# cambyse/po-rrt

Measured on NVIDIA B200. Metric: edge_world_validity_checks_per_s, higher is better.
Workload: dtype u8

## Files before the change

### po_rrt_b200/csrc/common.cuh

```cuda
#pragma once
#include <cuda_runtime.h>
#include <stdint.h>

#include <cstdio>
#include <cstring>
#include <string>
#include <vector>

#include "../../include/porrt_b200.h"

#define PORRT_API extern "C" __attribute__((visibility("default")))

struct DevBuf {
  void* p = nullptr;
  size_t cap = 0;
  cudaError_t ensure(size_t bytes) {
    if (bytes <= cap) return cudaSuccess;
    if (p) cudaFree(p);
    p = nullptr; cap = 0;
    size_t want = bytes + bytes / 4 + 256;
    cudaError_t e = cudaMalloc(&p, want);
    if (e == cudaSuccess) cap = want;
    return e;
  }
  cudaError_t grow_keep(size_t bytes, size_t keep_bytes, cudaStream_t st) {
    if (bytes <= cap) return cudaSuccess;
    void* q = nullptr;
    const size_t want = bytes + bytes / 2 + 256;
    cudaError_t e = cudaMalloc(&q, want);
    if (e != cudaSuccess) return e;
    if (p && keep_bytes) {
      e = cudaMemcpyAsync(q, p, keep_bytes, cudaMemcpyDeviceToDevice, st);
      if (e == cudaSuccess) e = cudaStreamSynchronize(st);
      if (e != cudaSuccess) { cudaFree(q); return e; }
    }
    if (p) cudaFree(p);
    p = q; cap = want;
    return cudaSuccess;
  }
  void release() { if (p) cudaFree(p); p = nullptr; cap = 0; }
  template <class T> T* as() const { return (T*)p; }
};

struct PinBuf {
  void* p = nullptr;
  size_t cap = 0;
  cudaError_t ensure(size_t bytes) {
    if (bytes <= cap) return cudaSuccess;
    if (p) cudaFreeHost(p);
    p = nullptr; cap = 0;
    size_t want = bytes + bytes / 4 + 256;
    cudaError_t e = cudaHostAlloc(&p, want, cudaHostAllocDefault);
    if (e == cudaSuccess) cap = want;
    return e;
  }
  void release() { if (p) cudaFreeHost(p); p = nullptr; cap = 0; }
  template <class T> T* as() const { return (T*)p; }
};

struct MapDev {
  const uint8_t* grid;
  const uint8_t* coarse;
  int32_t coarse_cw;
  const uint32_t* plane;
  const uint32_t* bits;
  int32_t plane_cw, plane_ch;
  int32_t plane_bytes;
  int32_t plane_guard;
  int32_t bits_var_words;
  int32_t H, W;
  int32_t tiles_x;
  int32_t kind;
  int32_t free_vid;
  int32_t mask_words;
  double low0, low1, ppm, hm1;
};

static const int MAX_SLOTS = 3;

struct porrt_ctx {
  int device = 0;
  int sm_count = 148;
  cudaStream_t stream = nullptr;
  cudaStream_t own_stream = nullptr;
  cudaStream_t copy_in = nullptr, copy_out = nullptr;
  cudaEvent_t ev_in[MAX_SLOTS] = {}, ev_k[MAX_SLOTS] = {}, ev_out[MAX_SLOTS] = {};
  std::string err;
  int64_t launches = 0;
  cudaEvent_t ev_t[16] = {};
  int n_marks = 0, n_last = 0;
  double last_ms[16] = {};

  bool has_map = false;
  MapDev map = {};
  int n_zones = 0, n_worlds = 0, n_validities = 0, mask_words = 1;
  double visibility = 0.0;
  std::vector<uint64_t> validities;
  std::vector<double> zone_pos;
  std::vector<uint64_t> zone_world_masks;
  DevBuf d_grid, d_coarse, d_validities, d_zone_pos, d_plane, d_bits;
  bool force_large_map_path = false;
  bool force_global_sweeps = false;

  int64_t n_vertices = 0;
  bool grid_stale = false;
  double cell_request = 0.0;
  double cell = 0, inv_cell = 0, org_x = 0, org_y = 0;
  int32_t cells_x = 0, cells_y = 0;
  DevBuf d_vxy_sorted, d_vid_sorted, d_cell_start, d_vxy, d_vcell;
  DevBuf nn_tmp[3];
  DevBuf d_nbr_start, d_nbr_script;
  bool nbr_ready = false;
  DevBuf nn_stage;
  DevBuf comm_tmp;
  DevBuf nn_stage2;
  int32_t nn_fb_n = 0;
  int32_t reach_words = 1;

  struct BeliefState_ {
    int64_t V = 0; int32_t B = 0, n_worlds = 0;
    std::vector<int64_t> row_ptr; std::vector<int32_t> col, edge_vid; std::vector<double> xy;
    std::vector<double> beliefs;
    const double* dist = nullptr; const uint8_t* type = nullptr;
    std::vector<uint8_t> exists;
    std::vector<int32_t> node_obs_set;
    std::vector<int64_t> succ_ptr;
    std::vector<int32_t> succ_belief;
    std::vector<uint8_t> compat;
    int32_t n_validities = 0;
    bool on_host = false;
    DevBuf dev;
    const double* d_dist_cm = nullptr; const uint8_t* d_type_cm = nullptr; const uint8_t* d_type = nullptr; const int32_t* d_colpos = nullptr;
    std::vector<int32_t> colpos;
    std::vector<std::vector<double>> col_dist;
    std::vector<std::vector<uint8_t>> col_type;
  } bel;
  std::vector<int32_t> bel_node_vid;
  DevBuf d_bel_succ;
  int64_t prm_n = 0, prm_edges = 0;
  const int64_t* prm_row_ptr = nullptr;
  const int32_t* prm_col = nullptr;
  const void* radii_ptr = nullptr; int64_t radii_lo = 0, radii_n = 0; double radii_ms = 0, radii_sr = 0;
  DevBuf d_prm_row, d_prm_col;

  struct MmPrm_ {
    std::vector<int64_t> row_ptr; std::vector<int32_t> col, belief_id; std::vector<uint8_t> type;
  } mm;

  void* comm = nullptr;
  int comm_rank = 0, comm_world = 1;

  DevBuf kd_buf;
  cudaStream_t aux_stream = nullptr;
  DevBuf scratch[12];
  PinBuf pin[6];
  PinBuf pin_flags;
};

#define CTX_CHECK(ctx) do { if (!(ctx)) return PORRT_ERR_INVALID_ARG; } while (0)

static inline int32_t porrt_fail(porrt_ctx* ctx, int32_t code, const std::string& msg) {
  if (ctx) ctx->err = msg;
  return code;
}

#define CUDA_TRY(ctx, expr)                                                                        \
  do {                                                                                             \
    cudaError_t _e = (expr);                                                                       \
    if (_e != cudaSuccess) {                                                                       \
      char _b[512];                                                                                \
      snprintf(_b, sizeof(_b), "%s:%d %s -> %s", __FILE__, __LINE__, #expr, cudaGetErrorString(_e)); \
      return porrt_fail(ctx, PORRT_ERR_CUDA, _b);                                                  \
    }                                                                                              \
  } while (0)

#define LAUNCH_CHECK(ctx)                                                                          \
  do {                                                                                             \
    (ctx)->launches += 1;                                                                          \
    CUDA_TRY(ctx, cudaGetLastError());                                                             \
  } while (0)

static inline bool is_pinned_host(const void* p) {
  cudaPointerAttributes a;
  if (cudaPointerGetAttributes(&a, p) != cudaSuccess) { cudaGetLastError(); return false; }
  return a.type == cudaMemoryTypeHost;
}

static inline void tstart(porrt_ctx* ctx) { ctx->n_marks = 0; if (ctx->ev_t[0]) cudaEventRecord(ctx->ev_t[ctx->n_marks++], ctx->stream); }
static inline void tmark(porrt_ctx* ctx) { if (ctx->ev_t[0] && ctx->n_marks < 16) cudaEventRecord(ctx->ev_t[ctx->n_marks++], ctx->stream); }
static inline void tfinish(porrt_ctx* ctx) {
  ctx->n_last = 0;
  for (int k = 0; k + 1 < ctx->n_marks; ++k) {
    float ms = 0.f;
    if (cudaEventElapsedTime(&ms, ctx->ev_t[k], ctx->ev_t[k + 1]) != cudaSuccess) { cudaGetLastError(); ms = -1.f; }
    ctx->last_ms[ctx->n_last++] = ms;
  }
}

static inline int div_up(int64_t a, int64_t b) { return (int)((a + b - 1) / b); }

void comm_shard_range(int64_t n, int rank, int world, int64_t* lo, int64_t* hi);
int32_t comm_all_gatherv_dev(porrt_ctx* ctx, const void* send_dev, void* recv_dev, const int64_t* offsets , cudaStream_t st);
struct EdgeOut {
  int32_t* vid = nullptr;
  int8_t* vid8 = nullptr;
  uint64_t* mask = nullptr;
};
int32_t map_edge_validity_dev(porrt_ctx* ctx, const double* from_dev, const double* to_dev, int64_t n,
                              int32_t* out_vid_dev, uint64_t* out_mask_dev, cudaStream_t st);
int32_t map_edge_launch(porrt_ctx* ctx, const double* from_dev, const double* to_dev, const int32_t* from_idx_dev,
                        const int32_t* to_idx_dev, int64_t n, const EdgeOut& out, cudaStream_t st);
int32_t map_edge_validity_indexed_dev(porrt_ctx* ctx, const double* xy_dev, const int32_t* from_idx_dev, const int32_t* to_idx_dev,
                                      int64_t n, int32_t* out_vid_dev, cudaStream_t st);
int32_t edge3_build(porrt_ctx* ctx, cudaStream_t st);
bool edge3_usable(const porrt_ctx* ctx);
int32_t edge3_launch(porrt_ctx* ctx, const double* from_dev, const double* to_dev, int64_t n, const EdgeOut& out,
                     const int32_t* from_idx_dev, const int32_t* to_idx_dev, cudaStream_t st);
struct GridDev;
bool nn_tile_usable(const porrt_ctx* ctx, int64_t m);
int32_t nn_tile_radius_collect(porrt_ctx* ctx, const GridDev& g, const double* q_dev, const double* radius_dev, int64_t m,
                               const uint32_t* prefix_dev, const uint64_t* reach_dev, const uint32_t* world_dev, int32_t* counts_dev,
                               int64_t* stg_off_dev, const int32_t** staging_out, const int32_t** fb_list_out, int32_t* fb_n_out,
                               int64_t* staged_total_out = nullptr);
int32_t nn_tile_radius_place(porrt_ctx* ctx, const int32_t* staging, const int64_t* stg_off_dev, const int64_t* offsets_dev, int64_t m,
                             int32_t* ids_dev);
int32_t nn_tile_knn(porrt_ctx* ctx, const GridDev& g, const double* q_dev, int64_t m, int k, const uint64_t* reach_dev,
                    const uint32_t* world_dev, int32_t* ids_dev, double* dist_dev, int32_t* ties_dev, const int32_t** fb_list_out,
                    int32_t* fb_n_out);
int32_t nn_vertices_set_dev(porrt_ctx* ctx, const double* xy_dev, int64_t n, double cell_size, const double* lo, const double* hi);
int32_t nn_flush_appended(porrt_ctx* ctx);
int32_t nn_radius_count_fill_dev(porrt_ctx* ctx, const double* q_dev, const double* radius_dev, int64_t m,
                                 const uint32_t* prefix_dev, const uint64_t* reach_dev, const uint32_t* world_dev,
                                 int64_t* offsets_dev , DevBuf* ids_buf, int64_t* total_out,
                                 const uint32_t* prefix_lo_dev = nullptr, bool sort_ids = false, bool allow_tiles = true);
int32_t scan_exclusive_i64(porrt_ctx* ctx, const int32_t* counts_dev, int64_t n, int64_t* out_dev );
int32_t read_flags_dev(porrt_ctx* ctx, const int32_t* flags_dev, int n, int32_t* out, cudaStream_t st);
int32_t segments_sort_by_key_dev(porrt_ctx* ctx, const int64_t* offsets_dev, int64_t m, int32_t* ids_dev,
                                 const int32_t* key_of_id_dev, int64_t key_limit, const int32_t* seg_list_dev = nullptr, int64_t n_listed = 0);
int32_t radix_sort_pairs(porrt_ctx* ctx, uint64_t* keys, uint32_t* vals, int64_t n, int key_bits);
int bits_for(uint64_t max_value);
int32_t prm_build_impl(porrt_ctx* ctx, const double* samples_xy, int64_t n, double max_step, double search_radius,
                       const double* ms_arr, const double* sr_arr, int64_t* out_row_ptr, int32_t* out_col, int64_t cap,
                       int64_t* out_n_edges, double* out_phase_ms, const int64_t* group_ptr = nullptr, int32_t n_groups = 0);
int32_t kd_preorder_rank_dev(porrt_ctx* ctx, const double* xy_dev, int64_t n, int32_t* out_rank_dev, const uint32_t* root_of_dev = nullptr,
                             cudaStream_t st = nullptr, std::string* err = nullptr, int64_t* n_launch = nullptr);
```

### po_rrt_b200/csrc/ctx.cu

```cuda
#include <ctype.h>
#include <sched.h>

#include <cstdlib>

#include "common.cuh"

PORRT_API const char* porrt_version(void) { return "porrt_b200 0.1 (sm_100a)"; }

PORRT_API int32_t porrt_ctx_create(int32_t device, porrt_ctx** out_ctx) {
  if (!out_ctx) return PORRT_ERR_INVALID_ARG;
  *out_ctx = nullptr;
  int count = 0;
  if (cudaGetDeviceCount(&count) != cudaSuccess || count == 0 || device < 0 || device >= count) {
    cudaGetLastError();
    return PORRT_ERR_CUDA;
  }
  cudaDeviceProp prop;
  if (cudaGetDeviceProperties(&prop, device) != cudaSuccess) return PORRT_ERR_CUDA;
  if (prop.major != 10) return PORRT_ERR_UNSUPPORTED;
  if (cudaSetDevice(device) != cudaSuccess) return PORRT_ERR_CUDA;
  porrt_ctx* ctx = new porrt_ctx();
  ctx->device = device;
  ctx->sm_count = prop.multiProcessorCount;
  int prio_least = 0, prio_greatest = 0;
  cudaDeviceGetStreamPriorityRange(&prio_least, &prio_greatest);
  bool ok = cudaStreamCreateWithPriority(&ctx->own_stream, cudaStreamNonBlocking, prio_least) == cudaSuccess &&
            cudaStreamCreateWithPriority(&ctx->aux_stream, cudaStreamNonBlocking, prio_greatest) == cudaSuccess &&
            cudaStreamCreateWithFlags(&ctx->copy_in, cudaStreamNonBlocking) == cudaSuccess &&
            cudaStreamCreateWithFlags(&ctx->copy_out, cudaStreamNonBlocking) == cudaSuccess;
  for (int s = 0; ok && s < MAX_SLOTS; ++s)
    ok = cudaEventCreateWithFlags(&ctx->ev_in[s], cudaEventDisableTiming) == cudaSuccess &&
         cudaEventCreateWithFlags(&ctx->ev_k[s], cudaEventDisableTiming) == cudaSuccess &&
         cudaEventCreateWithFlags(&ctx->ev_out[s], cudaEventDisableTiming) == cudaSuccess;
  for (int s = 0; ok && s < 16; ++s) ok = cudaEventCreate(&ctx->ev_t[s]) == cudaSuccess;
  if (!ok) { cudaGetLastError(); porrt_ctx_destroy(ctx); return PORRT_ERR_CUDA; }
  ctx->stream = ctx->own_stream;
  *out_ctx = ctx;
  return PORRT_OK;
}

PORRT_API int32_t porrt_ctx_destroy(porrt_ctx* ctx) {
  CTX_CHECK(ctx);
  cudaSetDevice(ctx->device);
  cudaDeviceSynchronize();
  porrt_comm_destroy(ctx);
  ctx->d_grid.release(); ctx->d_coarse.release(); ctx->d_validities.release(); ctx->d_zone_pos.release();
  ctx->d_plane.release(); ctx->d_bits.release();
  ctx->d_vxy_sorted.release(); ctx->d_vid_sorted.release(); ctx->d_cell_start.release();
  ctx->d_vxy.release(); ctx->d_vcell.release();
  for (DevBuf& b : ctx->nn_tmp) b.release();
  ctx->nn_stage.release(); ctx->nn_stage2.release(); ctx->comm_tmp.release(); ctx->d_nbr_start.release(); ctx->d_nbr_script.release();
  for (DevBuf& b : ctx->scratch) b.release();
  ctx->kd_buf.release(); ctx->d_prm_row.release(); ctx->d_prm_col.release(); ctx->d_bel_succ.release(); ctx->bel.dev.release();
  if (ctx->aux_stream) cudaStreamDestroy(ctx->aux_stream);
  for (PinBuf& b : ctx->pin) b.release();
  ctx->pin_flags.release();
  for (int s = 0; s < MAX_SLOTS; ++s) {
    if (ctx->ev_in[s]) cudaEventDestroy(ctx->ev_in[s]);
    if (ctx->ev_k[s]) cudaEventDestroy(ctx->ev_k[s]);
    if (ctx->ev_out[s]) cudaEventDestroy(ctx->ev_out[s]);
  }
  for (int s = 0; s < 16; ++s) if (ctx->ev_t[s]) cudaEventDestroy(ctx->ev_t[s]);
  if (ctx->own_stream) cudaStreamDestroy(ctx->own_stream);
  if (ctx->copy_in) cudaStreamDestroy(ctx->copy_in);
  if (ctx->copy_out) cudaStreamDestroy(ctx->copy_out);
  delete ctx;
  return PORRT_OK;
}

PORRT_API int32_t porrt_ctx_set_stream(porrt_ctx* ctx, void* cuda_stream) {
  CTX_CHECK(ctx);
  ctx->stream = cuda_stream ? (cudaStream_t)cuda_stream : ctx->own_stream;
  return PORRT_OK;
}

PORRT_API int32_t porrt_ctx_synchronize(porrt_ctx* ctx) {
  CTX_CHECK(ctx);
  CUDA_TRY(ctx, cudaSetDevice(ctx->device));
  CUDA_TRY(ctx, cudaStreamSynchronize(ctx->stream));
  return PORRT_OK;
}

PORRT_API int32_t porrt_ctx_bind_host_thread(porrt_ctx* ctx, int32_t* out_node) {
  CTX_CHECK(ctx);
  if (out_node) *out_node = -1;
  char bus[32] = {0};
  CUDA_TRY(ctx, cudaDeviceGetPCIBusId(bus, sizeof(bus), ctx->device));
  for (char* c = bus; *c; ++c) *c = (char)tolower(*c);
  char path[160];
  snprintf(path, sizeof(path), "/sys/bus/pci/devices/%s/numa_node", bus);
  FILE* f = fopen(path, "r");
  if (!f) return PORRT_OK;
  int node = -1;
  if (fscanf(f, "%d", &node) != 1) node = -1;
  fclose(f);
  if (node < 0) return PORRT_OK;
  snprintf(path, sizeof(path), "/sys/devices/system/node/node%d/cpulist", node);
  f = fopen(path, "r");
  if (!f) return PORRT_OK;
  char list[4096] = {0};
  const bool got = fgets(list, sizeof(list), f) != nullptr;
  fclose(f);
  if (!got) return PORRT_OK;
  cpu_set_t set;
  CPU_ZERO(&set);
  int n_cpus = 0;
  for (char* tok = strtok(list, ",\n"); tok; tok = strtok(nullptr, ",\n")) {
    int a = 0, b = 0;
    const int k = sscanf(tok, "%d-%d", &a, &b);
    if (k == 1) b = a;
    if (k < 1) continue;
    for (int c = a; c <= b && c < CPU_SETSIZE; ++c) { CPU_SET(c, &set); ++n_cpus; }
  }
  if (n_cpus == 0) return PORRT_OK;
  cpu_set_t cur, both;
  if (sched_getaffinity(0, sizeof(cur), &cur) == 0) {
    CPU_AND(&both, &set, &cur);
    if (CPU_COUNT(&both) == 0) return PORRT_OK;
    set = both;
  }
  if (sched_setaffinity(0, sizeof(set), &set) != 0) return PORRT_OK;
  if (out_node) *out_node = node;
  return PORRT_OK;
}

PORRT_API const char* porrt_last_error(porrt_ctx* ctx) { return ctx ? ctx->err.c_str() : "null ctx"; }
PORRT_API int64_t porrt_ctx_launch_count(porrt_ctx* ctx) { return ctx ? ctx->launches : 0; }

PORRT_API int32_t porrt_ctx_last_phase_ms(porrt_ctx* ctx, double* out_ms, int32_t cap, int32_t* out_n) {
  CTX_CHECK(ctx);
  int n = ctx->n_last < cap ? ctx->n_last : cap;
  for (int k = 0; k < n; ++k) out_ms[k] = ctx->last_ms[k];
  if (out_n) *out_n = n;
  return PORRT_OK;
}
```

### po_rrt_b200/csrc/edge3.cu

```cuda
#include "edge_common.cuh"

struct Rec3 {
  int32_t lo_raw0;
  int32_t idx0;
  int32_t stride_major;
  int32_t stride_minor;
  int32_t n0m;
  int32_t dxo;
  uint32_t S;
  int32_t n_strips;
  int32_t c0, n0;
  int32_t dirs;
  int32_t pad;
};

struct WarpMem {
  uint4 rec[3][32];
  uint32_t obst[32];
  uint32_t zmin[32], zmax[32];
  uint32_t qb[E3_QB];
  uint32_t qg[E3_QG];
};

template <int KIND, bool INDEXED>
__global__ void __launch_bounds__(E3_MAX_WARPS * 32, 1)
edge_validity_v3_kernel(MapDev m, const double2* __restrict__ from, const double2* __restrict__ to, int64_t n,
                        int32_t* __restrict__ out_vid, int8_t* __restrict__ out_vid8, uint64_t* __restrict__ out_mask,
                        const uint64_t* __restrict__ validities, const int32_t* __restrict__ from_idx,
                        const int32_t* __restrict__ to_idx) {
  extern __shared__ __align__(128) unsigned char smem[];
  uint64_t* s_mbar = (uint64_t*)(smem + m.plane_bytes);
  const int lane = threadIdx.x & 31, wib = threadIdx.x >> 5;
  WarpMem& wm = *(WarpMem*)(smem + m.plane_bytes + 16 + (size_t)wib * sizeof(WarpMem));
  const uint32_t lt_mask = (1u << lane) - 1u;

  if (threadIdx.x == 0) {
    asm volatile("mbarrier.init.shared::cta.b64 [%0], 1;" ::"r"(smem_u32(s_mbar)));
    asm volatile("fence.mbarrier_init.release.cluster;" ::: "memory");
  }
  __syncthreads();
  if (threadIdx.x == 0) {
    asm volatile("mbarrier.arrive.expect_tx.shared::cta.b64 _, [%0], %1;" ::"r"(smem_u32(s_mbar)), "r"((uint32_t)m.plane_bytes) : "memory");
    for (int off = 0; off < m.plane_bytes; off += 32768) {
      const int sz = min(32768, m.plane_bytes - off);
      asm volatile("cp.async.bulk.shared::cluster.global.mbarrier::complete_tx::bytes [%0], [%1], %2, [%3];" ::"r"(smem_u32(smem + off)),
                   "l"((const unsigned char*)m.plane + off), "r"((uint32_t)sz), "r"(smem_u32(s_mbar))
                   : "memory");
    }
  }
  bool plane_ready = false;

  const int64_t n_warps = (int64_t)gridDim.x * (blockDim.x >> 5);
  const int64_t warp = (int64_t)blockIdx.x * (blockDim.x >> 5) + wib;
  const int cw = m.plane_cw, ch = m.plane_ch;
  int qb_n = 0, qg_n = 0;

  auto drain = [&]() {
    __syncwarp();
#if !E3_ITEM_QUEUE
    int live_n = 0;
    for (int q0 = 0; q0 < qb_n; q0 += 32) {
      const int q = q0 + lane;
      uint32_t ent = 0;
      bool live = false;
      if (q < qb_n) { ent = wm.qb[q]; live = wm.obst[ent & 31] == 0; }
      const unsigned lv = __ballot_sync(0xffffffffu, live);
      __syncwarp();
      if (live) wm.qb[live_n + __popc(lv & lt_mask)] = ent;
      live_n += __popc(lv);
      __syncwarp();
    }
    for (int q0 = 0; q0 < live_n; q0 += 32) {
      const int q = q0 + lane;
      if (q < live_n) {
        const uint32_t ent = wm.qb[q];
        const int e = ent & 31, ts = (int)(ent >> 5);
#else
    for (int i0 = 0; i0 < qb_n; i0 += 32) {
      uint32_t i_ent = 0, i_want = 0;
      if (i0 + lane < qb_n) {
        i_ent = wm.qb[2 * (i0 + lane)]; i_want = wm.qb[2 * (i0 + lane) + 1];
        if (wm.obst[i_ent & 31] != 0) i_want = 0;
      }
      const int i_cnt = __popc(i_want);
      int i_incl = i_cnt;
#pragma unroll
      for (int o = 1; o < 32; o <<= 1) {
        const int t = __shfl_up_sync(0xffffffffu, i_incl, o);
        if (lane >= o) i_incl += t;
      }
      const int live_n = __shfl_sync(0xffffffffu, i_incl, 31);
      uint32_t* qs = wm.qb + 2 * E3_QI;
      for (int pos = i_incl - i_cnt; i_want; i_want &= i_want - 1)
        qs[pos++] = i_ent + ((uint32_t)((__ffs(i_want) - 1) >> 2) << 5);
      __syncwarp();
    for (int q0 = 0; q0 < live_n; q0 += 32) {
      const int q = q0 + lane;
      if (q < live_n) {
        const uint32_t ent = qs[q];
        const int e = ent & 31, ts = (int)(ent >> 5);
#endif
        if (wm.obst[e] == 0) {
          const uint4 r0 = wm.rec[0][e], r1 = wm.rec[1][e];
          const int dirs = (int)wm.rec[2][e].z;
          const int dxo = (int)r1.y, n0m = (int)r1.x;
          const uint32_t S = r1.z;
          const int lo_raw = (int)r0.x + ts * E3_BS;
          const int k_lo = max(0, lo_raw), k_hi = min(dxo, lo_raw + E3_BS - 1);
          const bool neg_major = (dirs & 2) != 0;
          const int bn_a = minor_m((uint32_t)k_lo, S, n0m) >> E3_LOG_BS;
          const int bn_b = minor_m((uint32_t)k_hi, S, n0m) >> E3_LOG_BS;
          const int blk_a = (int)r0.y - m.plane_guard + ts * (int)r0.z + bn_a * (int)r0.w;
          const uint32_t* tiles = m.bits + (size_t)(((dirs & 1) << 1) | ((dirs >> 2) & 1)) * (size_t)m.bits_var_words;
          uint32_t A[8], B[8];
#pragma unroll
          for (int w = 0; w < 8; ++w) B[w] = 0;
          ld256(A, tiles + (size_t)blk_a * 8);
          if (bn_b != bn_a) ld256(B, tiles + (size_t)(blk_a + (int)r0.w) * 8);
          const int k0 = neg_major ? lo_raw + E3_BS - 1 : lo_raw;
          const int c_hi = n0m - (bn_a << E3_LOG_BS);
          const int t_lo = neg_major ? lo_raw + E3_BS - 1 - k_hi : k_lo - lo_raw;
          const int t_hi = neg_major ? lo_raw + E3_BS - 1 - k_lo : k_hi - lo_raw;
          const uint32_t Vm = ((2u << t_hi) - 1u) & ~((1u << t_lo) - 1u);
          uint32_t acc = 0;
#if !E3_FINE_MODE
          uint64_t Y = ((uint64_t)(uint32_t)c_hi << 32) + (uint64_t)((int64_t)k0 * (int64_t)(uint64_t)S) + E3_BIAS;
          const uint64_t D = (neg_major ? (uint64_t)0 - (uint64_t)S : (uint64_t)S) - (1ull << 32);
#endif
#pragma unroll
          for (int t = 0; t < E3_BS; ++t) {
            const uint32_t V = (t & 1) ? __byte_perm(A[t >> 1], B[t >> 1], 0x7632) : __byte_perm(A[t >> 1], B[t >> 1], 0x5410);
#if E3_FINE_MODE
            int kt;
            asm("mad.lo.s32 %0, %1, %2, %3;" : "=r"(kt) : "r"(neg_major ? -1 : 1), "r"(t), "r"(k0));
            const int u = minor_m((uint32_t)kt, S, c_hi);
            if (Vm & (1u << t)) acc |= (1u << u) & V;
#else
            const uint32_t x = Vm & (1u << t);
            acc |= __funnelshift_l(x, x, (uint32_t)(Y >> 32)) & V;
            Y += D;
#endif
          }
          if (acc) wm.obst[e] = 1;
        }
      }
      __syncwarp();
    }
#if E3_ITEM_QUEUE
    }
#endif
    for (int q0 = 0; q0 < qg_n; q0 += 2) {
      const int q = q0 + (lane >> 4);
      uint32_t code = 255;
      int e = 0;
      if (q < qg_n) {
        const uint32_t ent = wm.qg[q];
        e = ent & 31;
        const int ts = (int)(ent >> 5);
        const uint4 r0 = wm.rec[0][e], r1 = wm.rec[1][e], r2 = wm.rec[2][e];
        const int dirs = (int)r2.z, dxo = (int)r1.y;
        const int lo_raw = (int)r0.x + ts * E3_BS;
        const int k = max(0, lo_raw) + (lane & 15);
        if (k <= min(dxo, lo_raw + E3_BS - 1)) {
          const int mk = minor_m((uint32_t)k, r1.z, 0);
          const int major = (int)r2.x + ((dirs & 2) ? -k : k), minor = (int)r2.y + ((dirs & 4) ? -mk : mk);
          const int i = (dirs & 1) ? major : minor, j = (dirs & 1) ? minor : major;
          code = __ldg(m.grid + tile_addr(i, j, m.tiles_x));
        }
      }
      const bool blocking = KIND == PORRT_DOMAIN_SHELF ? code != 255 : code == 0;
      const bool gray = KIND != PORRT_DOMAIN_SHELF && code != 0 && code != 255;
      const unsigned half_mask = 0xffffu << (lane & 16);
      const unsigned bl = __ballot_sync(0xffffffffu, blocking) & half_mask;
      const unsigned gr_all = __ballot_sync(0xffffffffu, gray);
      if (gr_all) {
        uint32_t zmin = gray ? code : 255u, zmax = gray ? code : 0u;
#pragma unroll
        for (int o = 8; o; o >>= 1) {
          zmin = min(zmin, __shfl_xor_sync(0xffffffffu, zmin, o));
          zmax = max(zmax, __shfl_xor_sync(0xffffffffu, zmax, o));
        }
        if ((gr_all & half_mask) && (lane & 15) == 0) { atomicMin(&wm.zmin[e], zmin); atomicMax(&wm.zmax[e], zmax); }
      }
      if (bl && (lane & 15) == 0) wm.obst[e] = 1;
    }
    __syncwarp();
    qb_n = 0; qg_n = 0;
  };

  for (int64_t base = warp * 32; base < n; base += n_warps * 32) {
    const int64_t eidx = base + lane;
    if (!plane_ready) { mbar_wait0(s_mbar); plane_ready = true; }
    int my_flags = 0;
    uint32_t pre_blocked = 0;
    int c0 = 0, n0 = 0, dxo = 0, dyo = 0, dirs = 0, n_strips = 0;
    uint4 r0 = make_uint4(0, 0, 0, 0);
    uint32_t S = 0;
    int n0m = 0;
    if (eidx < n) {
      const double2 a = INDEXED ? from[from_idx[eidx]] : from[eidx];
      const double2 b = INDEXED ? to[to_idx[eidx]] : to[eidx];
      uint32_t ai, aj, bi, bj;
      to_pixel(m, a.x, a.y, ai, aj);
      to_pixel(m, b.x, b.y, bi, bj);
      my_flags = ((ai >= (uint32_t)m.H || aj >= (uint32_t)m.W) ? 1 : 0) | ((bi >= (uint32_t)m.H || bj >= (uint32_t)m.W) ? 2 : 0);
      const int di = (int)bi - (int)ai, dj = (int)bj - (int)aj;
      const int adi = abs(di), adj = abs(dj);
      const bool major_i = adi >= adj;
      dxo = major_i ? adi : adj; dyo = major_i ? adj : adi;
      const int d_major = major_i ? di : dj, d_minor = major_i ? dj : di;
      c0 = major_i ? (int)ai : (int)aj; n0 = major_i ? (int)aj : (int)ai;
      dirs = (major_i ? 1 : 0) | (d_major < 0 ? 2 : 0) | (d_minor < 0 ? 4 : 0);
      if (!my_flags) {
        const int sb = m.plane_guard + ((int)ai >> E3_LOG_BS) * cw + ((int)aj >> E3_LOG_BS);
        const uint32_t sc = plane_class<false>(smem, (uint32_t)sb);
        pre_blocked = sc == K_BLOCKED ? 1u : 0u;
#if E3_START_PIXEL
        if (sc == K_MIXED || sc == K_SPECIAL) {
          const uint32_t code = __ldg(m.grid + tile_addr((int)ai, (int)aj, m.tiles_x));
          pre_blocked = (KIND == PORRT_DOMAIN_SHELF ? code != 255 : code == 0) ? 1u : 0u;
        }
#endif
      }
      if (!my_flags && !pre_blocked) {
        if (dxo > 0) S = slope_fixed_point(dyo, dxo);
        const int sgn = (dirs & 2) ? -1 : 1;
        const int b0 = c0 >> E3_LOG_BS, b1 = (c0 + sgn * dxo) >> E3_LOG_BS;
        n_strips = (b1 > b0 ? b1 - b0 : b0 - b1) + 1;
        const int blocks_minor = major_i ? cw : ch;
        int stride_minor = major_i ? 1 : cw;
        int idx0 = m.plane_guard + b0 * (major_i ? cw : 1);
        n0m = n0;
        if (dirs & 4) { n0m = blocks_minor * E3_BS - 1 - n0; idx0 += (blocks_minor - 1) * stride_minor; stride_minor = -stride_minor; }
        r0.x = (uint32_t)(sgn * ((b0 << E3_LOG_BS) - c0) - ((dirs & 2) ? E3_BS - 1 : 0));
        r0.y = (uint32_t)idx0;
        r0.z = (uint32_t)(sgn * (major_i ? cw : 1));
        r0.w = (uint32_t)stride_minor;
      }
    }
    wm.rec[0][lane] = r0;
    wm.rec[1][lane] = make_uint4((uint32_t)n0m, (uint32_t)dxo, S, (uint32_t)n_strips);
    wm.rec[2][lane] = make_uint4((uint32_t)c0, (uint32_t)n0, (uint32_t)dirs, 0u);
    wm.obst[lane] = pre_blocked; wm.zmin[lane] = 255; wm.zmax[lane] = 0;
    const int my_items = (n_strips + E3_G - 1) / E3_G;
    auto process_item = [&](const int e, const int item, const bool has_item) {
      uint32_t cls = 0;
      const int ts0 = has_item ? item * E3_G : 0;
      {
        const uint4 q0 = wm.rec[0][e], q1 = wm.rec[1][e];
        const int sm_ = (int)q0.z, sn_ = (int)q0.w, e_dxo = (int)q1.y, e_n0m = (int)q1.x;
        const uint32_t e_S = q1.z;
        const int left = has_item ? (int)q1.w - ts0 : 0;
        int lo_raw = (int)q0.x + ts0 * E3_BS;
        int idx_m = (int)q0.y + ts0 * sm_;
#pragma unroll
        for (int g = 0; g < E3_G; ++g) {
          const int k_lo = g == 0 ? max(0, lo_raw) : lo_raw, k_hi = min(e_dxo, lo_raw + E3_BS - 1);
          const uint32_t na = (uint32_t)minor_m((uint32_t)k_lo, e_S, e_n0m), nb = (uint32_t)minor_m((uint32_t)k_hi, e_S, e_n0m);
          const uint32_t ia = (uint32_t)idx_m + shr_c<E3_SHR_FMA != 0>(na, E3_LOG_BS) * (uint32_t)sn_;
          const uint32_t ib = (uint32_t)idx_m + shr_c<E3_SHR_FMA != 0>(nb, E3_LOG_BS) * (uint32_t)sn_;
          const uint32_t ca = plane_class<(E3_ADDR_MODE & 1) != 0>(smem, ia), cb = plane_class<(E3_ADDR_MODE & 2) != 0>(smem, ib);
          cls += ((1u << ca) | (1u << cb)) * (1u << (4 * g));
          lo_raw += E3_BS; idx_m += sm_;
        }
        cls &= left >= E3_G ? 0xffffffffu : ((1u << (4 * max(left, 0))) - 1u);
      }
      const uint32_t blocked = cls & 0x44444444u, special = (cls >> 3) & 0x11111111u;
      if (blocked) wm.obst[e] = 1;
      const uint32_t want = blocked ? 0u : ((cls >> 1) & 0x11111111u & ~special);
#if E3_ITEM_QUEUE
      {
        const unsigned bal = __ballot_sync(0xffffffffu, want != 0);
        if (bal) {
          if (want) {
            const int pos = 2 * (qb_n + __popc(bal & lt_mask));
            wm.qb[pos] = (uint32_t)e | ((uint32_t)ts0 << 5);
            wm.qb[pos + 1] = want;
          }
          qb_n += __popc(bal);
        }
      }
#else
      if (__any_sync(0xffffffffu, want != 0)) {
        const int cnt = __popc(want);
        int sc = cnt;
#pragma unroll
        for (int o = 1; o < 32; o <<= 1) {
          const int t = __shfl_up_sync(0xffffffffu, sc, o);
          if (lane >= o) sc += t;
        }
        int pb = qb_n + sc - cnt;
        qb_n += __shfl_sync(0xffffffffu, sc, 31);
        const uint32_t ent0 = (uint32_t)e | ((uint32_t)ts0 << 5);
#pragma unroll
        for (int g = 0; g < E3_G; ++g)
          if (want & (1u << (4 * g))) wm.qb[pb++] = ent0 + ((uint32_t)g << 5);
      }
#endif
      if (__any_sync(0xffffffffu, special != 0)) {
#pragma unroll
        for (int g = 0; g < E3_G; ++g) {
          const unsigned bal = __ballot_sync(0xffffffffu, (special >> (4 * g)) & 1u);
          if ((special >> (4 * g)) & 1u) wm.qg[qg_n + __popc(bal & lt_mask)] = (uint32_t)e | ((uint32_t)(ts0 + g) << 5);
          qg_n += __popc(bal);
        }
      }
    };
#if E3_TWO_PHASE
    const bool may_overflow = true;
    __syncwarp();
    process_item(lane, 0, my_items > 0);
    __syncwarp();
#if E3_TWO_PHASE == 2
    if (__any_sync(0xffffffffu, my_items > 1) && (qb_n | qg_n)) drain();
#endif
    int rem = (my_items <= 1 || wm.obst[lane] != 0) ? 0 : my_items - 1;
    int incl = rem;
#pragma unroll
    for (int o = 1; o < 32; o <<= 1) {
      const int t = __shfl_up_sync(0xffffffffu, incl, o);
      if (lane >= o) incl += t;
    }
    const int total = __shfl_sync(0xffffffffu, incl, 31);
    for (int w0 = 0; w0 < total; w0 += 32) {
      if (may_overflow && (qb_n > E3_QB_LIMIT || qg_n > E3_QG - 32 * E3_G)) drain();
      const int w = w0 + lane;
      int e = 0;
#pragma unroll
      for (int sft = 16; sft >= 1; sft >>= 1) {
        const int v = __shfl_sync(0xffffffffu, incl, e + sft - 1);
        if (v <= w) e += sft;
      }
      const int excl = __shfl_sync(0xffffffffu, incl - rem, e);
      process_item(e, 1 + w - excl, w < total);
      __syncwarp();
    }
#else
    int incl = max(1, my_items);
#pragma unroll
    for (int o = 1; o < 32; o <<= 1) {
      const int t = __shfl_up_sync(0xffffffffu, incl, o);
      if (lane >= o) incl += t;
    }
    const int total = __shfl_sync(0xffffffffu, incl, 31);
    const bool may_overflow = total * E3_G > min(E3_QB, E3_QG);
    __syncwarp();
    for (int w0 = 0; w0 < total; w0 += 32) {
      if (may_overflow && (qb_n > E3_QB_LIMIT || qg_n > E3_QG - 32 * E3_G)) drain();
      const int d = incl - w0;
      const int e_base = __popc(__ballot_sync(0xffffffffu, d <= 0));
      const unsigned marks = __reduce_or_sync(0xffffffffu, (d >= 1 && d <= 32) ? (1u << (d - 1)) : 0u);
      const int e = min(31, e_base + __popc(marks & lt_mask));
      const int p_prev = __shfl_sync(0xffffffffu, incl, (e + 31) & 31);
      process_item(e, w0 + lane - (e ? p_prev : 0), w0 + lane < total);
      __syncwarp();
    }
#endif
    if (qb_n | qg_n) drain();
    __syncwarp();

    if (eidx < n) {
      int32_t r;
      bool slow = false;
      if (my_flags & 1) r = PORRT_PANIC_OOB;
      else if (my_flags & 2) slow = true;
      else {
        const bool is_blocked = wm.obst[lane] != 0;
        if (KIND == PORRT_DOMAIN_SHELF) r = is_blocked ? R_BLOCKED : R_FREE;
        else {
          const uint32_t zmin = wm.zmin[lane], zmax = wm.zmax[lane];
          if (zmax != 0 && (zmin != zmax || zmax == 254)) slow = true;
          else r = is_blocked ? R_BLOCKED : (zmax ? (int32_t)zmin - 1 : R_FREE);
        }
      }
      if (slow) {
        Walker wk;
        const int sm = (dirs & 2) ? -1 : 1, sn = (dirs & 4) ? -1 : 1;
        wk.dxo = dxo; wk.dyo = dyo;
        wk.M = dxo > 1 ? (0xFFFFFFFFFFFFFFFFull / (uint64_t)dxo) + 1ull : 0ull;
        if (dirs & 1) { wk.ai = c0; wk.aj = n0; wk.ui = sm; wk.uj = 0; wk.vi = 0; wk.vj = sn; }
        else { wk.ai = n0; wk.aj = c0; wk.ui = 0; wk.uj = sm; wk.vi = sn; wk.vj = 0; }
        r = walk_sequential<KIND>(m, wk);
        if (KIND == PORRT_DOMAIN_SHELF && r == R_LOW) r = R_BLOCKED;
      }
      store_edge_result(m, eidx, walk_to_validity(m, r), out_vid, out_vid8, out_mask, validities);
    }
    __syncwarp();
  }
  if (!plane_ready) mbar_wait0(s_mbar);
}

template <int KIND>
__global__ void __launch_bounds__(256) edge3_build_kernel(const uint8_t* __restrict__ grid, int H, int W, int tiles_x, int cw, int ch,
                                                          uint32_t* __restrict__ plane, int guard, uint16_t* __restrict__ bits, size_t var_halfwords) {
  const int lane = threadIdx.x & 31, half = lane >> 4, r = lane & 15;
  const int64_t pair = ((int64_t)blockIdx.x * blockDim.x + threadIdx.x) >> 5;
  const int64_t n_blocks = (int64_t)cw * ch;
  const int64_t blk = pair * 2 + half;
  const bool have = blk < n_blocks;
  const int bi = have ? (int)(blk / cw) : 0, bj = have ? (int)(blk % cw) : 0;
  const int i = bi * E3_BS + r;
  uint32_t rowmask = 0, n_in = 0, n_block = 0, n_special = 0;
  if (have && i < H) {
#pragma unroll
    for (int c = 0; c < E3_BS; ++c) {
      const int j = bj * E3_BS + c;
      if (j < W) {
        const uint32_t code = grid[tile_addr(i, j, tiles_x)];
        ++n_in;
        const bool blocking = KIND == PORRT_DOMAIN_SHELF ? code != 255 : code == 0;
        if (blocking) { rowmask |= 1u << c; ++n_block; }
        else if (code != 255) ++n_special;
      }
    }
  }
  uint32_t colvec = 0;
#pragma unroll
  for (int c = 0; c < E3_BS; ++c) {
    const uint32_t bal = __ballot_sync(0xffffffffu, (rowmask >> c) & 1u);
    if (r == c) colvec = (bal >> (16 * half)) & 0xffffu;
  }
  uint32_t cnt = n_in | (n_block << 10) | (n_special << 20);
#pragma unroll
  for (int o = 8; o; o >>= 1) cnt += __shfl_xor_sync(0xffffffffu, cnt, o);
  if (have) {
    uint16_t* t0 = bits + (size_t)blk * 16 + r;
    t0[0] = (uint16_t)colvec;
    t0[var_halfwords] = (uint16_t)(__brev(colvec) >> 16);
    t0[2 * var_halfwords] = (uint16_t)rowmask;
    t0[3 * var_halfwords] = (uint16_t)(__brev(rowmask) >> 16);
    if (r == 0) {
      const uint32_t t_in = cnt & 1023u, t_block = (cnt >> 10) & 1023u, t_special = cnt >> 20;
      const uint32_t cls = t_special ? K_SPECIAL : (t_block == 0 ? K_FREE : (t_block == t_in ? K_BLOCKED : K_MIXED));
      const int64_t pb = blk + guard;
      if (cls) atomicOr(&plane[pb >> 4], cls << ((pb & 15) << 1));
    }
  }
}

int32_t edge3_build(porrt_ctx* ctx, cudaStream_t st) {
  MapDev& m = ctx->map;
  const int cw = (m.W + E3_BS - 1) / E3_BS, ch = (m.H + E3_BS - 1) / E3_BS;
  const size_t n_blocks = (size_t)cw * ch;
  const int guard = (int)(((size_t)(E3_G + 1) * cw + 63) / 64 * 64);
  const size_t plane_bytes = ((((n_blocks + 2 * (size_t)guard + 15) / 16) * 4 + 15) / 16) * 16;
  CUDA_TRY(ctx, ctx->d_plane.ensure(plane_bytes));
  CUDA_TRY(ctx, ctx->d_bits.ensure(n_blocks * 32 * 4));
  CUDA_TRY(ctx, cudaMemsetAsync(ctx->d_plane.p, 0, plane_bytes, st));
  const int grid = div_up((int64_t)((n_blocks + 1) / 2) * 32, 256);
  if (m.kind == PORRT_DOMAIN_SHELF)
    edge3_build_kernel<PORRT_DOMAIN_SHELF><<<grid, 256, 0, st>>>(m.grid, m.H, m.W, m.tiles_x, cw, ch, ctx->d_plane.as<uint32_t>(), guard, ctx->d_bits.as<uint16_t>(), n_blocks * 16);
  else
    edge3_build_kernel<PORRT_DOMAIN_DOOR><<<grid, 256, 0, st>>>(m.grid, m.H, m.W, m.tiles_x, cw, ch, ctx->d_plane.as<uint32_t>(), guard, ctx->d_bits.as<uint16_t>(), n_blocks * 16);
  LAUNCH_CHECK(ctx);
  m.plane = ctx->d_plane.as<uint32_t>();
  m.bits = ctx->d_bits.as<uint32_t>();
  m.plane_cw = cw;
  m.plane_ch = ch;
  m.plane_guard = guard;
  m.plane_bytes = (int32_t)plane_bytes;
  m.bits_var_words = (int32_t)(n_blocks * 8);
  return PORRT_OK;
}

static const int E3_SMEM_LIMIT = 227 * 1024;

static int edge3_max_warps(const porrt_ctx* ctx) {
  const int64_t room = (int64_t)E3_SMEM_LIMIT - ctx->map.plane_bytes - 16;
  const int64_t w = room / (int64_t)sizeof(WarpMem);
  return (int)(w > E3_MAX_WARPS ? E3_MAX_WARPS : w);
}

bool edge3_usable(const porrt_ctx* ctx) {
  return ctx->map.plane != nullptr && edge3_max_warps(ctx) >= 8 && ctx->map.H <= 32768 && ctx->map.W <= 32768;
}

template <int KIND, bool INDEXED>
static int32_t edge3_launch_t(porrt_ctx* ctx, const double2* from, const double2* to, int64_t n, const EdgeOut& out,
                              const int32_t* from_idx, const int32_t* to_idx, cudaStream_t st) {
  auto kern = edge_validity_v3_kernel<KIND, INDEXED>;
  static bool attr_set[16] = {};
  if (!attr_set[ctx->device & 15]) {
    CUDA_TRY(ctx, cudaFuncSetAttribute(kern, cudaFuncAttributeMaxDynamicSharedMemorySize, E3_SMEM_LIMIT));
    attr_set[ctx->device & 15] = true;
  }
  const int max_warps = edge3_max_warps(ctx);
  const int64_t warps_needed = (n + 31) / 32;
  int warps = (int)((warps_needed + ctx->sm_count - 1) / ctx->sm_count);
  warps = warps < 4 ? 4 : (warps > max_warps ? max_warps : warps);
  int64_t ctas = (warps_needed + warps - 1) / warps;
  if (ctas > ctx->sm_count) ctas = ctx->sm_count;
  const size_t smem = (size_t)ctx->map.plane_bytes + 16 + (size_t)warps * sizeof(WarpMem);
  kern<<<(int)ctas, warps * 32, smem, st>>>(ctx->map, from, to, n, out.vid, out.vid8, out.mask, ctx->d_validities.as<uint64_t>(), from_idx, to_idx);
  LAUNCH_CHECK(ctx);
  return PORRT_OK;
}

int32_t edge3_launch(porrt_ctx* ctx, const double* from_dev, const double* to_dev, int64_t n, const EdgeOut& out,
                     const int32_t* from_idx_dev, const int32_t* to_idx_dev, cudaStream_t st) {
  const double2* f = (const double2*)from_dev;
  const double2* t = (const double2*)to_dev;
  const bool shelf = ctx->map.kind == PORRT_DOMAIN_SHELF;
  if (from_idx_dev)
    return shelf ? edge3_launch_t<PORRT_DOMAIN_SHELF, true>(ctx, f, t, n, out, from_idx_dev, to_idx_dev, st)
                 : edge3_launch_t<PORRT_DOMAIN_DOOR, true>(ctx, f, t, n, out, from_idx_dev, to_idx_dev, st);
  return shelf ? edge3_launch_t<PORRT_DOMAIN_SHELF, false>(ctx, f, t, n, out, nullptr, nullptr, st)
               : edge3_launch_t<PORRT_DOMAIN_DOOR, false>(ctx, f, t, n, out, nullptr, nullptr, st);
}
```

### po_rrt_b200/csrc/edge_common.cuh

```cuda
#pragma once
#include "map_dev.cuh"

#ifndef E3_SHR_FMA
#define E3_SHR_FMA 0
#endif
#ifndef E3_ADDR_MODE
#define E3_ADDR_MODE 0
#endif
#ifndef E3_FINE_MODE
#define E3_FINE_MODE 0
#endif
#ifndef E3_START_PIXEL
#define E3_START_PIXEL 0
#endif
#ifndef E3_TWO_PHASE
#define E3_TWO_PHASE 1
#endif
#define E3_LOG_BS 4
#define E3_BS 16
#ifndef E3_G
#define E3_G 7
#endif
#define E3_QB 512
#define E3_QG 256
#ifndef E3_ITEM_QUEUE
#define E3_ITEM_QUEUE 1
#endif
#define E3_QI ((E3_QB - 32 * 8) / 2)
#if E3_ITEM_QUEUE
#define E3_QB_LIMIT (E3_QI - 32)
#else
#define E3_QB_LIMIT (E3_QB - 32 * E3_G)
#endif
#define E3_BIAS 65536ull
#ifndef E3_MAX_WARPS
#define E3_MAX_WARPS 32
#endif

#define K_FREE 0u
#define K_MIXED 1u
#define K_BLOCKED 2u
#define K_SPECIAL 3u

#ifndef E3_SLOPE_DIV
#define E3_SLOPE_DIV 0
#endif
__device__ __forceinline__ uint32_t slope_fixed_point(int dy, int dx) {
#if E3_SLOPE_DIV
  if (dy == dx) return 0xFFFFFFFFu;
  const uint32_t d = (uint32_t)dx, num = (uint32_t)dy << 16;
  const uint32_t q1 = num / d, r1 = num - q1 * d;
  return (q1 << 16) + ((r1 << 16) / d);
#else
  return __double2uint_rz(__dmul_rn(__dmul_rn((double)dy, 4294967296.0), __drcp_rn((double)dx)));
#endif
}

__device__ __forceinline__ int32_t minor_m(uint32_t k, uint32_t S, int32_t n0m) {
  return (int32_t)(((uint64_t)k * (uint64_t)S + (((uint64_t)(uint32_t)n0m << 32) | E3_BIAS)) >> 32);
}


template <bool FMA>
__device__ __forceinline__ uint32_t shr_c(uint32_t x, int s) { return FMA ? __umulhi(x, 1u << (32 - s)) : x >> s; }

template <bool WORD>
__device__ __forceinline__ uint32_t plane_class(const unsigned char* plane, uint32_t idx) {
  if (WORD) {
    const uint32_t w = ((const uint32_t*)plane)[__umulhi(idx, 1u << 28)];
    return __funnelshift_r(w, w, idx * 2u) & 3u;
  }
  return ((uint32_t)plane[idx >> 2] >> ((idx * 2u) & 6u)) & 3u;
}

__device__ __forceinline__ void ld256(uint32_t (&v)[8], const uint32_t* p) {
  asm volatile("ld.global.nc.v8.u32 {%0,%1,%2,%3,%4,%5,%6,%7}, [%8];"
               : "=r"(v[0]), "=r"(v[1]), "=r"(v[2]), "=r"(v[3]), "=r"(v[4]), "=r"(v[5]), "=r"(v[6]), "=r"(v[7])
               : "l"(p));
}

__device__ __forceinline__ uint32_t smem_u32(const void* p) { return (uint32_t)__cvta_generic_to_shared(p); }

__device__ __forceinline__ void mbar_wait0(uint64_t* bar) {
  uint32_t done = 0;
  while (!done)
    asm volatile("{ .reg .pred p; mbarrier.try_wait.parity.shared::cta.b64 p, [%1], 0; selp.u32 %0, 1, 0, p; }"
                 : "=r"(done) : "r"(smem_u32(bar)) : "memory");
}
```

Baseline: 1602 billion.

## Use atomic ticket work-stealing for edge batches and split sparse tail rows

Replaces the static grid-stride loop over 32-edge batches with dynamic scheduling. Each warp fetches its next batch from a global atomic ticket counter, using per-launch slots with a host-tracked base so the counter never needs a reset. When fewer than 16 fine-tile items remain in the drain queue, two lanes now share each item: each loads half of the 256-bit tile and scans half the rows, to cut tail imbalance. This adds one global atomic per batch per warp plus a memset at map setup, and also adds optional counting instrumentation.

```diff
diff --git a/po_rrt_b200/csrc/common.cuh b/po_rrt_b200/csrc/common.cuh
--- a/po_rrt_b200/csrc/common.cuh
+++ b/po_rrt_b200/csrc/common.cuh
@@ -99,6 +99,9 @@
   std::vector<double> zone_pos;
   std::vector<uint64_t> zone_world_masks;
   DevBuf d_grid, d_coarse, d_validities, d_zone_pos, d_plane, d_bits;
+  DevBuf d_e3_ticket;
+  uint64_t e3_launches = 0;
+  unsigned long long e3_ticket_base[64] = {};
   bool force_large_map_path = false;
   bool force_global_sweeps = false;
 
diff --git a/po_rrt_b200/csrc/ctx.cu b/po_rrt_b200/csrc/ctx.cu
--- a/po_rrt_b200/csrc/ctx.cu
+++ b/po_rrt_b200/csrc/ctx.cu
@@ -45,7 +45,7 @@
   cudaDeviceSynchronize();
   porrt_comm_destroy(ctx);
   ctx->d_grid.release(); ctx->d_coarse.release(); ctx->d_validities.release(); ctx->d_zone_pos.release();
-  ctx->d_plane.release(); ctx->d_bits.release();
+  ctx->d_plane.release(); ctx->d_bits.release(); ctx->d_e3_ticket.release();
   ctx->d_vxy_sorted.release(); ctx->d_vid_sorted.release(); ctx->d_cell_start.release();
   ctx->d_vxy.release(); ctx->d_vcell.release();
   for (DevBuf& b : ctx->nn_tmp) b.release();
diff --git a/po_rrt_b200/csrc/edge3.cu b/po_rrt_b200/csrc/edge3.cu
--- a/po_rrt_b200/csrc/edge3.cu
+++ b/po_rrt_b200/csrc/edge3.cu
@@ -22,12 +22,17 @@
   uint32_t qg[E3_QG];
 };
 
+#if E3_COUNT
+__device__ unsigned long long e3_counts[3];
+#endif
+
 template <int KIND, bool INDEXED>
 __global__ void __launch_bounds__(E3_MAX_WARPS * 32, 1)
 edge_validity_v3_kernel(MapDev m, const double2* __restrict__ from, const double2* __restrict__ to, int64_t n,
                         int32_t* __restrict__ out_vid, int8_t* __restrict__ out_vid8, uint64_t* __restrict__ out_mask,
                         const uint64_t* __restrict__ validities, const int32_t* __restrict__ from_idx,
-                        const int32_t* __restrict__ to_idx) {
+                        const int32_t* __restrict__ to_idx, unsigned long long* __restrict__ ticket,
+                        const unsigned long long ticket_base) {
   extern __shared__ __align__(128) unsigned char smem[];
   uint64_t* s_mbar = (uint64_t*)(smem + m.plane_bytes);
   const int lane = threadIdx.x & 31, wib = threadIdx.x >> 5;
@@ -71,6 +76,7 @@
       __syncwarp();
     }
     for (int q0 = 0; q0 < live_n; q0 += 32) {
+      const bool split = false;
       const int q = q0 + lane;
       if (q < live_n) {
         const uint32_t ent = wm.qb[q];
@@ -90,12 +96,16 @@
         if (lane >= o) i_incl += t;
       }
       const int live_n = __shfl_sync(0xffffffffu, i_incl, 31);
+#if E3_COUNT
+      if (lane == 0) atomicAdd(&e3_counts[2], (unsigned long long)live_n);
+#endif
       uint32_t* qs = wm.qb + 2 * E3_QI;
       for (int pos = i_incl - i_cnt; i_want; i_want &= i_want - 1)
         qs[pos++] = i_ent + ((uint32_t)((__ffs(i_want) - 1) >> 2) << 5);
       __syncwarp();
     for (int q0 = 0; q0 < live_n; q0 += 32) {
-      const int q = q0 + lane;
+      const bool split = live_n - q0 <= 16;
+      const int q = split ? q0 + (lane >> 1) : q0 + lane;
       if (q < live_n) {
         const uint32_t ent = qs[q];
         const int e = ent & 31, ts = (int)(ent >> 5);
@@ -112,17 +122,36 @@
           const int bn_b = minor_m((uint32_t)k_hi, S, n0m) >> E3_LOG_BS;
           const int blk_a = (int)r0.y - m.plane_guard + ts * (int)r0.z + bn_a * (int)r0.w;
           const uint32_t* tiles = m.bits + (size_t)(((dirs & 1) << 1) | ((dirs >> 2) & 1)) * (size_t)m.bits_var_words;
-          uint32_t A[8], B[8];
-#pragma unroll
-          for (int w = 0; w < 8; ++w) B[w] = 0;
-          ld256(A, tiles + (size_t)blk_a * 8);
-          if (bn_b != bn_a) ld256(B, tiles + (size_t)(blk_a + (int)r0.w) * 8);
           const int k0 = neg_major ? lo_raw + E3_BS - 1 : lo_raw;
           const int c_hi = n0m - (bn_a << E3_LOG_BS);
           const int t_lo = neg_major ? lo_raw + E3_BS - 1 - k_hi : k_lo - lo_raw;
           const int t_hi = neg_major ? lo_raw + E3_BS - 1 - k_lo : k_hi - lo_raw;
           const uint32_t Vm = ((2u << t_hi) - 1u) & ~((1u << t_lo) - 1u);
           uint32_t acc = 0;
+          if (split) {
+            const int p = lane & 1;
+            uint32_t A[4], B[4];
+#pragma unroll
+            for (int w = 0; w < 4; ++w) B[w] = 0;
+            ld128(A, tiles + (size_t)blk_a * 8 + 4 * p);
+            if (bn_b != bn_a) ld128(B, tiles + (size_t)(blk_a + (int)r0.w) * 8 + 4 * p);
+            const uint32_t Vp = Vm >> (8 * p);
+            const int k0p = k0 + (neg_major ? -8 : 8) * p;
+            uint64_t Y = ((uint64_t)(uint32_t)c_hi << 32) + (uint64_t)((int64_t)k0p * (int64_t)(uint64_t)S) + E3_BIAS;
+            const uint64_t D = (neg_major ? (uint64_t)0 - (uint64_t)S : (uint64_t)S) - (1ull << 32);
+#pragma unroll
+            for (int t = 0; t < E3_BS / 2; ++t) {
+              const uint32_t V = (t & 1) ? __byte_perm(A[t >> 1], B[t >> 1], 0x7632) : __byte_perm(A[t >> 1], B[t >> 1], 0x5410);
+              const uint32_t x = Vp & (1u << t);
+              acc |= __funnelshift_l(x, x, (uint32_t)(Y >> 32)) & V;
+              Y += D;
+            }
+          } else {
+          uint32_t A[8], B[8];
+#pragma unroll
+          for (int w = 0; w < 8; ++w) B[w] = 0;
+          ld256(A, tiles + (size_t)blk_a * 8);
+          if (bn_b != bn_a) ld256(B, tiles + (size_t)(blk_a + (int)r0.w) * 8);
 #if !E3_FINE_MODE
           uint64_t Y = ((uint64_t)(uint32_t)c_hi << 32) + (uint64_t)((int64_t)k0 * (int64_t)(uint64_t)S) + E3_BIAS;
           const uint64_t D = (neg_major ? (uint64_t)0 - (uint64_t)S : (uint64_t)S) - (1ull << 32);
@@ -140,6 +169,7 @@
             acc |= __funnelshift_l(x, x, (uint32_t)(Y >> 32)) & V;
             Y += D;
 #endif
+          }
           }
           if (acc) wm.obst[e] = 1;
         }
@@ -188,7 +218,10 @@
     qb_n = 0; qg_n = 0;
   };
 
-  for (int64_t base = warp * 32; base < n; base += n_warps * 32) {
+  for (int64_t batch = warp; batch * 32 < n;) {
+    const int64_t base = batch * 32;
+    unsigned long long next = 0;
+    if (lane == 0) next = atomicAdd(ticket, 1ull) - ticket_base;
     const int64_t eidx = base + lane;
     if (!plane_ready) { mbar_wait0(s_mbar); plane_ready = true; }
     int my_flags = 0;
@@ -268,6 +301,13 @@
       const uint32_t blocked = cls & 0x44444444u, special = (cls >> 3) & 0x11111111u;
       if (blocked) wm.obst[e] = 1;
       const uint32_t want = blocked ? 0u : ((cls >> 1) & 0x11111111u & ~special);
+#if E3_COUNT
+      {
+        const int slots = __popc(__ballot_sync(0xffffffffu, has_item)) * E3_G;
+        const int queued = __reduce_add_sync(0xffffffffu, (unsigned)__popc(want));
+        if (lane == 0) { atomicAdd(&e3_counts[0], (unsigned long long)slots); atomicAdd(&e3_counts[1], (unsigned long long)queued); }
+      }
+#endif
 #if E3_ITEM_QUEUE
       {
         const unsigned bal = __ballot_sync(0xffffffffu, want != 0);
@@ -386,6 +426,7 @@
       store_edge_result(m, eidx, walk_to_validity(m, r), out_vid, out_vid8, out_mask, validities);
     }
     __syncwarp();
+    batch = n_warps + (int64_t)__shfl_sync(0xffffffffu, next, 0);
   }
   if (!plane_ready) mbar_wait0(s_mbar);
 }
@@ -460,6 +501,9 @@
   m.plane_guard = guard;
   m.plane_bytes = (int32_t)plane_bytes;
   m.bits_var_words = (int32_t)(n_blocks * 8);
+  CUDA_TRY(ctx, ctx->d_e3_ticket.ensure(E3_TICKET_SLOTS * sizeof(unsigned long long)));
+  CUDA_TRY(ctx, cudaMemsetAsync(ctx->d_e3_ticket.p, 0, E3_TICKET_SLOTS * sizeof(unsigned long long), st));
+  for (unsigned long long& b : ctx->e3_ticket_base) b = 0;
   return PORRT_OK;
 }
 
@@ -491,8 +535,21 @@
   int64_t ctas = (warps_needed + warps - 1) / warps;
   if (ctas > ctx->sm_count) ctas = ctx->sm_count;
   const size_t smem = (size_t)ctx->map.plane_bytes + 16 + (size_t)warps * sizeof(WarpMem);
-  kern<<<(int)ctas, warps * 32, smem, st>>>(ctx->map, from, to, n, out.vid, out.vid8, out.mask, ctx->d_validities.as<uint64_t>(), from_idx, to_idx);
+  const int slot = (int)(ctx->e3_launches++ & (E3_TICKET_SLOTS - 1));
+  unsigned long long* ticket = ctx->d_e3_ticket.as<unsigned long long>() + slot;
+  const unsigned long long ticket_base = ctx->e3_ticket_base[slot];
+  kern<<<(int)ctas, warps * 32, smem, st>>>(ctx->map, from, to, n, out.vid, out.vid8, out.mask, ctx->d_validities.as<uint64_t>(), from_idx, to_idx,
+                                            ticket, ticket_base);
   LAUNCH_CHECK(ctx);
+  ctx->e3_ticket_base[slot] += (unsigned long long)((n + 31) / 32);
+#if E3_COUNT
+  unsigned long long c[3];
+  CUDA_TRY(ctx, cudaStreamSynchronize(st));
+  CUDA_TRY(ctx, cudaMemcpyFromSymbol(c, e3_counts, sizeof(c)));
+  fprintf(stderr, "E3_COUNT edges %lld slots %llu bitmap_queued %llu bitmap_drained %llu\n", (long long)n, c[0], c[1], c[2]);
+  const unsigned long long zero[3] = {0, 0, 0};
+  CUDA_TRY(ctx, cudaMemcpyToSymbol(e3_counts, zero, sizeof(zero)));
+#endif
   return PORRT_OK;
 }
 
diff --git a/po_rrt_b200/csrc/edge_common.cuh b/po_rrt_b200/csrc/edge_common.cuh
--- a/po_rrt_b200/csrc/edge_common.cuh
+++ b/po_rrt_b200/csrc/edge_common.cuh
@@ -33,6 +33,7 @@
 #define E3_QB_LIMIT (E3_QB - 32 * E3_G)
 #endif
 #define E3_BIAS 65536ull
+#define E3_TICKET_SLOTS 64
 #ifndef E3_MAX_WARPS
 #define E3_MAX_WARPS 32
 #endif
@@ -73,6 +74,10 @@
   return ((uint32_t)plane[idx >> 2] >> ((idx * 2u) & 6u)) & 3u;
 }
 
+__device__ __forceinline__ void ld128(uint32_t (&v)[4], const uint32_t* p) {
+  asm volatile("ld.global.nc.v4.u32 {%0,%1,%2,%3}, [%4];" : "=r"(v[0]), "=r"(v[1]), "=r"(v[2]), "=r"(v[3]) : "l"(p));
+}
+
 __device__ __forceinline__ void ld256(uint32_t (&v)[8], const uint32_t* p) {
   asm volatile("ld.global.nc.v8.u32 {%0,%1,%2,%3,%4,%5,%6,%7}, [%8];"
                : "=r"(v[0]), "=r"(v[1]), "=r"(v[2]), "=r"(v[3]), "=r"(v[4]), "=r"(v[5]), "=r"(v[6]), "=r"(v[7])
```

New measurement: 1626 billion (median of 6 runs). +1.5%, better.
